# graphdeco-inria/editable-gaussian-reflections

Hardware: AMD Instinct MI355X
Metric: Mrays/s fwd+bwd @1080p, 1M Gaussians (higher is better)
Workload: dtype f32; 1 GPU; BASELINE config C: synthetic dense-init room+spheres cloud, HEADLINE variant = init (literal dense-init opacity 0.1 (config.py:44): Kc ~ 22 per ray, bounces mostly die), N=1000000, 1920x1080, one training iteration: export + update_bvh + forward + backward + grad import, num_bounces=2, jitter on, reference default config; variant=init, gaussians=1000000, width=1920, height=1080, parallelism=image tiles x1 + 1 all-reduce of the launch's [22N] gradients, team_help=product default (on)

## Files before the change

### editable-gaussian-reflections_amd/csrc/backward_chain.hpp

```cpp
#pragma once

constexpr int BOUNCE_QUEUE_FLOATS = 25 * EGR_WAVE;
static_assert(EGR_GT_STRIDE * EGR_GT_SLOTS >= BOUNCE_QUEUE_FLOATS, "the bounce queues must fit into the table");

template <int TEAM> struct BwdWave {
    int lane, wv;
    uint32_t *gt_keys;
    float *gt_vals;
    uint32_t *gt_claim;
    float4 *stage;
    BwdTeamShared<TEAM> &bteam;
    uint4 *bitems;
    float *bdl;
    float *bray;
    float exp_power;
    int num_bounces;
    float view_size;
    uint32_t bepoch;
    bool table_dirty;
};

struct BwdDiag {
    EGR_TIMES(unsigned long long bw_t0 = 0ull, bw_t1 = 0ull; uint32_t bw_rows0 = 0u;)
};

struct RayGrads {
    f3 dL_rgb, dL_n, dL_f0;
    float dL_depth, dL_rough;
    f3 ro, rd;
    f3 rem_rgb, rem_n, rem_f0;
    float rem_depth, rem_rough, T_minus_Ttot;
};

template <bool PRIMARY, bool BATCH, int TEAM>
EGR_DI RayGrads output_gradients(const DeviceView &v, const BwdWave<TEAM> &W, const ChainTask &task, const TaskGeom &tg, const StateRef &S, const int step,
                                 const uint32_t steps_done, const uint32_t nhits) {
    RayGrads g{mk3(0, 0, 0), mk3(0, 0, 0), mk3(0, 0, 0), 0.0f, 0.0f, mk3(0, 0, 0), mk3(0, 0, 1), mk3(0, 0, 0), mk3(0, 0, 0), mk3(0, 0, 0), 0.0f, 0.0f, 0.0f};
    if (nhits > 0) {
        const uint32_t pid = tg.pixel_id;
        const float third = 1.0f / 3.0f;
        if constexpr (PRIMARY) {
            f3 o_rgb = S.ld3(SF(0, S_RGB)), o_n = S.ld3(SF(0, S_NORMAL)), o_f0 = S.ld3(SF(0, S_F0));
            float o_depth = S.ld(SF(0, S_DEPTH)), o_rough = S.ld(SF(0, S_ROUGH));
            if constexpr (BATCH) {
                const size_t P = v.num_pixels;
                const uint32_t bframe = task.bframe;
                auto tgt = [&](int b, uint32_t ch, uint32_t c) { const float *p = v.batch_targets[b]; return p ? p[((size_t)bframe * ch + c) * P + pid] : 0.0f; };
                g.dL_rgb = mk3(third * sign1(o_rgb.x - tgt(0, 3, 0)), third * sign1(o_rgb.y - tgt(0, 3, 1)), third * sign1(o_rgb.z - tgt(0, 3, 2))) * *v.cfg.loss_weight_diffuse;
                g.dL_depth = sign1(o_depth - tgt(2, 1, 0)) * *v.cfg.loss_weight_depth;
                g.dL_n = mk3(third * sign1(o_n.x - tgt(3, 3, 0)), third * sign1(o_n.y - tgt(3, 3, 1)), third * sign1(o_n.z - tgt(3, 3, 2))) * *v.cfg.loss_weight_normal;
                g.dL_f0 = mk3(third * sign1(o_f0.x - tgt(5, 3, 0)), third * sign1(o_f0.y - tgt(5, 3, 1)), third * sign1(o_f0.z - tgt(5, 3, 2))) * *v.cfg.loss_weight_f0;
                g.dL_rough = sign1(o_rough - tgt(4, 1, 0)) * *v.cfg.loss_weight_roughness;
            } else {
                const bool planes = v.target_planes != 0u;
                const size_t cs = planes ? (size_t)v.num_pixels : (size_t)1;
                auto tgt = [&](int b, uint32_t ch, uint32_t c) { const float *p = v.batch_targets[b]; return p ? p[(size_t)pid * (planes ? 1u : ch) + c * cs] : 0.0f; };
                g.dL_rgb = mk3(third * sign1(o_rgb.x - tgt(0, 3, 0)), third * sign1(o_rgb.y - tgt(0, 3, 1)), third * sign1(o_rgb.z - tgt(0, 3, 2))) * *v.cfg.loss_weight_diffuse;
                g.dL_depth = sign1(o_depth - tgt(2, 1, 0)) * *v.cfg.loss_weight_depth;
                g.dL_n = mk3(third * sign1(o_n.x - tgt(3, 3, 0)), third * sign1(o_n.y - tgt(3, 3, 1)), third * sign1(o_n.z - tgt(3, 3, 2))) * *v.cfg.loss_weight_normal;
                g.dL_f0 = mk3(third * sign1(o_f0.x - tgt(5, 3, 0)), third * sign1(o_f0.y - tgt(5, 3, 1)), third * sign1(o_f0.z - tgt(5, 3, 2))) * *v.cfg.loss_weight_f0;
                g.dL_rough = sign1(o_rough - tgt(4, 1, 0)) * *v.cfg.loss_weight_roughness;
            }
            const PrimaryRay p = primary_ray<BATCH>(v, tg, task, W.view_size);
            g.ro = p.ro, g.rd = p.rd;
        } else {
            f3 spec = mk3(0, 0, 0);
            for (int j = 1; j < W.num_bounces + 1; j++)
                if ((uint32_t)j < steps_done) spec = spec + S.ld3(SF(j, S_RGB));
            f3 t_spec;
            if constexpr (BATCH) {
                const float *p = v.batch_targets[1];
                const size_t P = v.num_pixels, q = (size_t)task.bframe * 3 * P + pid;
                t_spec = p ? mk3(p[q], p[q + P], p[q + 2 * P]) : mk3(0, 0, 0);
            } else {
                const float *p = v.batch_targets[1];
                const size_t q = (size_t)pid * (v.target_planes ? 1u : 3u), cs = v.target_planes ? (size_t)v.num_pixels : (size_t)1;
                t_spec = p ? mk3(p[q], p[q + cs], p[q + 2 * cs]) : mk3(0, 0, 0);
            }
            float down = powf(1.0f - S.ld(SF(step - 1, S_ROUGH)), EGR_ROUGHNESS_DOWNWEIGHT_GRAD_POWER);
            g.dL_rgb = (mk3(third * sign1(spec.x - t_spec.x), third * sign1(spec.y - t_spec.y), third * sign1(spec.z - t_spec.z)) *
                        *v.cfg.loss_weight_specular) * down;
            g.dL_rgb = g.dL_rgb * S.ld3(SF(step - 1, S_THR));
            g.ro = S.ld3(SF(step - 1, S_NEXT_O));
            g.rd = S.ld3(SF(step - 1, S_NEXT_D));
        }
        g.rem_rgb = S.ld3(SF(step, S_REM_RGB)), g.rem_n = S.ld3(SF(step, S_REM_NORMAL)), g.rem_f0 = S.ld3(SF(step, S_REM_F0));
        g.rem_depth = S.ld(SF(step, S_REM_DEPTH)), g.rem_rough = S.ld(SF(step, S_REM_ROUGH));
        g.T_minus_Ttot = S.ld(SF(step, S_T)) - S.ld(SF(step, S_TTOT));
    }
    return g;
}

template <int TEAM> EGR_DI uint32_t bounce_hits(const DeviceView &v, BwdWave<TEAM> &W, const RayGrads &g, uint32_t blk, const uint32_t nhits, const uint32_t max_hits) {
    const int lane = W.lane, wv = W.wv;
    const float exp_power = W.exp_power;
    BwdTeamShared<TEAM> &bteam = W.bteam;
    uint4 *const bitems = W.bitems;
    float *const bdl = W.bdl, *const bray = W.bray;
    float4 *const stage = W.stage;
    const f3 dL_rgb = g.dL_rgb, ro = g.ro, rd = g.rd, rem_rgb = g.rem_rgb;
    const float T_minus_Ttot = g.T_minus_Ttot;
    uint32_t records = 0u;
    W.table_dirty = true;
    bdl[lane] = dL_rgb.x, bdl[EGR_WAVE + lane] = dL_rgb.y, bdl[2 * EGR_WAVE + lane] = dL_rgb.z;
    bray[lane] = ro.x, bray[EGR_WAVE + lane] = ro.y, bray[2 * EGR_WAVE + lane] = ro.z, bray[3 * EGR_WAVE + lane] = rd.x, bray[4 * EGR_WAVE + lane] = rd.y, bray[5 * EGR_WAVE + lane] = rd.z;
    f3 prev_rgb = mk3(0, 0, 0), w_rgb = mk3(0, 0, 0);
    const uint32_t nblocks = (max_hits + EGR_HIT_BLOCK_ROWS - 1) / EGR_HIT_BLOCK_ROWS;
    EGR_BWD_SYNC();
    for (uint32_t b = nblocks; b-- > 0;) {
        const float4 *rows = v.hit_arena + (size_t)blk * (EGR_HIT_BLOCK_ROWS + 1) * EGR_WAVE;
        for (int chunk = EGR_HIT_BLOCK_ROWS / 4 - 1; chunk >= 0; chunk--) {
            uint32_t nitems = 0u;
            float4 rec4[4], a04[4];
#pragma unroll
            for (int r4 = 0; r4 < 4; r4++) rec4[r4] = rows[(size_t)(1 + 4 * chunk + r4) * EGR_WAVE + lane];
#pragma unroll
            for (int r4 = 0; r4 < 4; r4++) a04[r4] = v.app[2 * ((b * EGR_HIT_BLOCK_ROWS + (uint32_t)(4 * chunk + r4)) < nhits ? f2u(rec4[r4].x) : 0u)];
#pragma unroll
            for (int r4 = 3; r4 >= 0; r4--) {
                const int row = 4 * chunk + r4;
                const uint32_t it = b * EGR_HIT_BLOCK_ROWS + (uint32_t)row;
                const bool act = it < nhits;
                float dL_dalpha = 0.0f, weight = 0.0f;
                uint32_t pos = 0u;
                if (act) {
                    const float4 rec = rec4[r4];
                    pos = f2u(rec.x);
                    const float alpha = rec.z, transmittance = rec.w;
                    weight = (float)((double)transmittance / (1.0 - (double)alpha) * (double)alpha);
                    const float4 a0 = a04[r4];
                    const f3 g_rgb = mk3(a0.x, a0.y, a0.z);
                    w_rgb = w_rgb + (g_rgb - prev_rgb) * transmittance;
                    prev_rgb = g_rgb;
                    const float one_m_alpha = 1.0f - alpha, r1ma = egr_rcp_refined(one_m_alpha);
                    const float tmp1 = egr_div_rn(1.0f, one_m_alpha, r1ma);
                    dL_dalpha += dot(w_rgb * tmp1, dL_rgb);
                    const float tmp2 = -egr_div_rn(T_minus_Ttot, one_m_alpha, r1ma);
                    dL_dalpha += tmp2 * dot(rem_rgb, dL_rgb);
                }
                const unsigned long long am = __ballot(act);
                if (act) bitems[nitems + __builtin_amdgcn_mbcnt_hi((uint32_t)(am >> 32), __builtin_amdgcn_mbcnt_lo((uint32_t)am, 0u))] = make_uint4((uint32_t)lane, f2u(dL_dalpha), pos, f2u(weight));
                nitems += (uint32_t)__popcll(am);
            }
            if (nitems == 0u) continue;
            EGR_BWD_SYNC();
            const uint32_t nbatch = (nitems + (uint32_t)EGR_WAVE - 1u) / (uint32_t)EGR_WAVE;
            if constexpr (TEAM > 1) {
                if (lane == 0) {
                    lds_poke(&bteam.finished[wv], 0u);
                    lds_poke(&bteam.nitems[wv], nitems);
                    W.bepoch = (W.bepoch + 1u) & 0xFFFu;
                    lds_poke(&bteam.ticket[wv], (W.bepoch << 20) | (nbatch << 10));
                }
                for (;;) {
                    uint32_t tk = 0u;
                    if (lane == 0) tk = atomicAdd(&bteam.ticket[wv], 1u);
                    tk = uniform_u32(tk);
                    const uint32_t bi = tk & 0x3FFu;
                    if (bi >= nbatch) break;
                    records += bounce_batch(v, exp_power, bitems, bdl, bray, bi * (uint32_t)EGR_WAVE, nitems, stage, lane);
                    if (lane == 0) atomicAdd(&bteam.finished[wv], 1u);
                }
                while (uniform_u32(lds_peek(&bteam.finished[wv])) < nbatch) __builtin_amdgcn_s_sleep(1);
            } else {
                for (uint32_t bi = 0; bi < nbatch; bi++) records += bounce_batch(v, exp_power, bitems, bdl, bray, bi * (uint32_t)EGR_WAVE, nitems, stage, lane);
            }
            EGR_BWD_SYNC();
        }
        blk = f2u(rows[0].x);
    }
    return records;
}

template <int TEAM> EGR_DI uint32_t primary_hits(const DeviceView &v, BwdWave<TEAM> &W, const RayGrads &g, uint32_t blk, const uint32_t nhits, const uint32_t max_hits) {
    const int lane = W.lane;
    uint32_t *const gt_keys = W.gt_keys, *const gt_claim = W.gt_claim;
    float *const gt_vals = W.gt_vals;
    float4 *const stage = W.stage;
    const f3 dL_rgb = g.dL_rgb, dL_n = g.dL_n, dL_f0 = g.dL_f0, ro = g.ro, rd = g.rd, rem_rgb = g.rem_rgb, rem_n = g.rem_n, rem_f0 = g.rem_f0;
    const float dL_depth = g.dL_depth, dL_rough = g.dL_rough, rem_depth = g.rem_depth, rem_rough = g.rem_rough, T_minus_Ttot = g.T_minus_Ttot;
    uint32_t records = 0u;
    f3 prev_rgb = mk3(0, 0, 0), w_rgb = mk3(0, 0, 0), prev_n = mk3(0, 0, 0), w_n = mk3(0, 0, 0), prev_f0 = mk3(0, 0, 0), w_f0 = mk3(0, 0, 0);
    float prev_rough = 0, w_rough = 0, prev_depth = 0, w_depth = 0;
    const uint32_t nblocks = (max_hits + EGR_HIT_BLOCK_ROWS - 1) / EGR_HIT_BLOCK_ROWS;
    EGR_STATS(unsigned long long bt_math = 0ull, bt_table = 0ull, bt_wide = 0ull, bt_rows = 0ull;)
    for (uint32_t b = nblocks; b-- > 0;) {
        const float4 *rows = v.hit_arena + (size_t)blk * (EGR_HIT_BLOCK_ROWS + 1) * EGR_WAVE;
        int pf_row = -1;
        float4 rec_pf = make_float4(0.f, 0.f, 0.f, 0.f);
        for (int row = EGR_HIT_BLOCK_ROWS - 1; row >= 0; row--) {
            const uint32_t it = b * EGR_HIT_BLOCK_ROWS + (uint32_t)row;
            if (it >= max_hits) continue;
            bool direct = false, want = false;
            uint32_t dpos = 0;
            float gx[EGR_GT_COMPS];
            EGR_STATS(const unsigned long long bt0 = __builtin_amdgcn_s_memtime(); unsigned long long bt1 = bt0; bt_rows++;)
            float4 rec_cur = rec_pf;
            const bool have_pf = pf_row == row;
            if (row > 0) {
                if (it <= nhits) rec_pf = rows[(size_t)row * EGR_WAVE + lane];
                pf_row = row - 1;
            }
            if (!have_pf) {
                if (it < nhits) rec_cur = rows[(size_t)(1 + row) * EGR_WAVE + lane];
#if defined(__HIP_DEVICE_COMPILE__)
                asm volatile("" ::"v"(rec_cur.x), "v"(rec_cur.y), "v"(rec_cur.z), "v"(rec_cur.w));
#endif
            }
            if (it < nhits) {
                const float4 rec = rec_cur;
                const uint32_t pos = f2u(rec.x);
                const float distance = rec.y, alpha = rec.z, transmittance = rec.w;
                const float4 a0 = v.app[2 * pos], a1 = v.app[2 * pos + 1], a2 = v.inst_w[4 * pos + 3];
                const f3 g_rgb = mk3(a0.x, a0.y, a0.z);
                const float weight = (float)((double)transmittance / (1.0 - (double)alpha) * (double)alpha);
                f3 d_rgb = (dL_rgb * weight);
                f3 d_n = dL_n * weight, d_f0 = dL_f0 * weight;
                float d_rough = dL_rough * weight;

                w_rgb = w_rgb + (g_rgb - prev_rgb) * transmittance;
                prev_rgb = g_rgb;
                {
                    f3 g_n = mk3(a0.w, a1.x, a1.y), g_f0 = mk3(a1.z, a1.w, a2.x);
                    w_n = w_n + (g_n - prev_n) * transmittance;
                    prev_n = g_n;
                    w_f0 = w_f0 + (g_f0 - prev_f0) * transmittance;
                    prev_f0 = g_f0;
                    w_rough += (a2.y - prev_rough) * transmittance;
                    prev_rough = a2.y;
                    w_depth += (distance - prev_depth) * transmittance;
                    prev_depth = distance;
                }
                float dL_dalpha = 0.0f;
                const float one_m_alpha = 1.0f - alpha, r1ma = egr_rcp_refined(one_m_alpha);
                const float tmp1 = egr_div_rn(1.0f, one_m_alpha, r1ma);
                dL_dalpha += dot(w_rgb * tmp1, dL_rgb);
                dL_dalpha += dot(w_n * tmp1, dL_n);
                dL_dalpha += dot(w_f0 * tmp1, dL_f0);
                dL_dalpha += (w_rough * tmp1) * dL_rough;
                dL_dalpha += (w_depth * tmp1) * dL_depth;
                const float tmp2 = -egr_div_rn(T_minus_Ttot, one_m_alpha, r1ma);
                dL_dalpha += tmp2 * dot(rem_rgb, dL_rgb);
                dL_dalpha += tmp2 * dot(rem_n, dL_n);
                dL_dalpha += tmp2 * dot(rem_f0, dL_f0);
                dL_dalpha += tmp2 * (rem_rough * dL_rough);
                dL_dalpha += tmp2 * (rem_depth * dL_depth);

                hit_geometry_fn(v, W.exp_power, pos, a2, ro, rd, dL_dalpha, gx);
                gx[PC_RGB] = d_rgb.x, gx[PC_RGB + 1] = d_rgb.y, gx[PC_RGB + 2] = d_rgb.z, gx[PC_WEIGHT] = weight;
                gx[PC_NORMAL] = d_n.x, gx[PC_NORMAL + 1] = d_n.y, gx[PC_NORMAL + 2] = d_n.z;
                gx[PC_F0] = d_f0.x, gx[PC_F0 + 1] = d_f0.y, gx[PC_F0 + 2] = d_f0.z, gx[PC_ROUGH] = d_rough;
                EGR_STATS(bt1 = __builtin_amdgcn_s_memtime();)
                dpos = pos;
                want = primary_presum(pos, gx, lane);
            }
            direct = primary_table_add(v, want, dpos, gx, gt_keys, gt_vals, gt_claim, stage, lane, records);
            EGR_STATS(const unsigned long long bt2 = __builtin_amdgcn_s_memtime(); bt_math += bt1 - bt0; bt_table += bt2 - bt1;)
            if (__ballot(direct) != 0ull) {
                float lo[EGR_REC0_COMPS], hi[EGR_REC1_COMPS];
#pragma unroll
                for (int c = 0; c < EGR_REC0_COMPS; c++) lo[c] = gx[c];
#pragma unroll
                for (int c = 0; c < EGR_REC1_COMPS; c++) hi[c] = gx[EGR_REC0_COMPS + c];
                wide_add_wave<EGR_REC0_CELL>(v, direct, dpos, lo, stage);
                wide_add_wave<EGR_REC1_CELL>(v, direct, dpos, hi, stage);
                records += 2u * (uint32_t)__popcll(__ballot(direct));
            }
            EGR_STATS(bt_wide += __builtin_amdgcn_s_memtime() - bt2;)
        }
        blk = f2u(rows[0].x);
    }
    EGR_STATS(const unsigned long long bt3 = __builtin_amdgcn_s_memtime();)
    records += grad_table_flush(v, gt_keys, gt_vals, stage, lane);
    EGR_STATS(if (lane == 0) {
        unsigned long long *d = diag64(v.control, DG_BWD_MATH_CYC);
        atomicAdd(d, bt_math), atomicAdd(d + 1, bt_table), atomicAdd(d + 2, bt_wide), atomicAdd(d + 3, __builtin_amdgcn_s_memtime() - bt3), atomicAdd(d + 4, bt_rows);
    })
    return records;
}

template <bool PRIMARY, int TEAM, bool BATCH> EGR_DI uint32_t backward_step(const DeviceView &v, BwdWave<TEAM> &W, const uint32_t tq, const int step, BwdDiag &D) {
    const int lane = W.lane;
    const uint32_t tqo = v.bwd_order[tq];
    const uint32_t blk = v.task_last_block[(size_t)step * (BATCH ? v.num_tasks * v.batch_frames : v.num_tasks) + tqo];
    if (blk == 0xFFFFFFFFu) return 0u;
    const ChainTask task = decode_task<BATCH>(v, tqo);
    const TaskGeom tg = task_geom(v, task.tb, lane);
    const StateRef S = state_of(v, task.tq, lane);
    const uint32_t steps_done = tg.inside ? f2u(S.ld(F_STEPS)) : 0u;
    const uint32_t nhits = (tg.inside && (uint32_t)step < steps_done && blk != 0xFFFFFFFFu) ? f2u(S.ld(SF(step, S_NHITS))) : 0u;
    const uint32_t max_hits = wave_max_u32(nhits);
    if (max_hits == 0) return 0u;
    EGR_TIMES_IS(8, if (PRIMARY) D.bw_rows0 = max_hits;)
    const RayGrads g = output_gradients<PRIMARY, BATCH>(v, W, task, tg, S, step, steps_done, nhits);
    if constexpr (PRIMARY) return primary_hits(v, W, g, blk, nhits, max_hits);
    else return bounce_hits(v, W, g, blk, nhits, max_hits);
}

template <int TEAM, bool BATCH> EGR_DI void backward_chain(const DeviceView v) {
    const int lane = threadIdx.x & (EGR_WAVE - 1);
    const int wv = __builtin_amdgcn_readfirstlane((int)(threadIdx.x >> 6));
    __shared__ uint32_t gt_keys_all[TEAM][EGR_GT_SLOTS];
    __shared__ __attribute__((aligned(16))) float gt_vals_all[TEAM][EGR_GT_STRIDE * EGR_GT_SLOTS];
    __shared__ uint32_t gt_claim_all[TEAM][EGR_GT_SLOTS];
    __shared__ float4 stage_all[TEAM][4 * EGR_WAVE];
    __shared__ BwdTeamShared<TEAM> bteam;
    if (threadIdx.x == 0) bteam.done = 0u;
    if (threadIdx.x < TEAM) bteam.ticket[threadIdx.x] = 0u, bteam.nitems[threadIdx.x] = 0u, bteam.finished[threadIdx.x] = 0u;
    uint32_t *const gt_keys = gt_keys_all[wv];
    float *const gt_vals = gt_vals_all[wv];
    for (int s = lane; s < EGR_GT_SLOTS; s += EGR_WAVE) gt_keys[s] = EGR_GT_EMPTY;
    for (int s = lane; s < EGR_GT_STRIDE * EGR_GT_SLOTS; s += EGR_WAVE) gt_vals[s] = 0.0f;
    __syncthreads();
    const float exp_power = *v.cfg.exp_power;
    const int num_bounces = min(*v.cfg.num_bounces, EGR_MAX_BOUNCES);
    const float view_size = BATCH ? 0.0f : tanf(*v.cam.vertical_fov_radians / 2.0f);
    BwdWave<TEAM> W{lane, wv, gt_keys, gt_vals, gt_claim_all[wv], stage_all[wv], bteam, reinterpret_cast<uint4 *>(gt_vals), gt_vals + 16 * EGR_WAVE, gt_vals + 19 * EGR_WAVE,
                    exp_power, num_bounces, view_size, 0u, false};
    uint32_t cur_q = blockIdx.x & 7u;
    uint32_t records = 0u;

    for (;;) {
        const uint32_t tq = wave_next_task(v.queues + 8 * EGR_QUEUE_STRIDE, BATCH ? v.num_tasks * v.batch_frames : v.num_tasks, cur_q, lane);
        if (tq == 0xFFFFFFFFu) break;
        BwdDiag D;
        EGR_TIMES_IS(8, D.bw_t0 = __builtin_amdgcn_s_memrealtime();)
        W.table_dirty = false;
        records += backward_step<true, TEAM, BATCH>(v, W, tq, 0, D);
        EGR_TIMES_IS(8, D.bw_t1 = __builtin_amdgcn_s_memrealtime();)
        for (int step = num_bounces; step >= 1; step--) records += backward_step<false, TEAM, BATCH>(v, W, tq, step, D);
        if (W.table_dirty) {
            EGR_BWD_SYNC();
            for (int s = lane; s < BOUNCE_QUEUE_FLOATS; s += EGR_WAVE) gt_vals[s] = 0.0f;
            EGR_BWD_SYNC();
        }
        EGR_TIMES_IS(8,
            const unsigned long long bw_t2 = __builtin_amdgcn_s_memrealtime();
            const TaskGeom btg = task_geom(v, decode_task<BATCH>(v, v.bwd_order[tq]).tb, lane);
            if (btg.inside) {
                if (lane == 0) v.stats.num_traversed_per_pixel[btg.pixel_id] = EGR_STAMP31(D.bw_t0), v.stats.num_accumulated_per_pixel[btg.pixel_id] = EGR_STAMP31(bw_t2);
                if (lane == 1) v.stats.num_traversed_per_pixel[btg.pixel_id] = EGR_STAMP31(D.bw_t1), v.stats.num_accumulated_per_pixel[btg.pixel_id] = (int32_t)D.bw_rows0;
            })
    }
    if constexpr (TEAM > 1) {
        if (lane == 0) atomicAdd(&bteam.done, 1u);
        records += bwd_team_help<TEAM>(v, exp_power, bteam, gt_vals_all, W.stage, wv, lane);
    }
    if (lane == 0 && records) atomicAdd(v.control + CW_BUCKET_RECORDS, records);
}
```

### editable-gaussian-reflections_amd/csrc/trace.hip

```cpp
#include <algorithm>
#include <cstdio>
#include <cstdlib>
#include <type_traits>
#include <utility>
#include <vector>

#define EGR_CONTRACT_AFTER_EPILOGUE
#include "egr_diag.hpp"
#include "egr_epilogue.hpp"

#ifndef EGR_GPOP
#define EGR_GPOP 5
#endif
#define EGR_WALK_MAX_LEAVES (8 * EGR_GPOP * EGR_WIDTH)
#define EGR_LBUF (64 + 2 * EGR_WALK_MAX_LEAVES)
#ifndef EGR_FPOP
#define EGR_FPOP 2
#endif
#ifndef EGR_PSTK
#define EGR_PSTK 512
#endif

namespace {

// ... 722 lines not shown
            float *cell = gt_vals + slot * EGR_GT_STRIDE;
            float cur[EGR_GT_COMPS];
#pragma unroll
            for (int c = 0; c < EGR_GT_COMPS; c++) cur[c] = cell[c];
#pragma unroll
            for (int c = 0; c < EGR_GT_COMPS; c++) cell[c] = cur[c] + gx[c];
            pending = false;
        }
        EGR_BWD_SYNC();
    }
    return want && !found;
}

struct ChainVec { double x, y, z; };
EGR_DI void scale_rot_chain(const float4 &M0, const float4 &M1, const float4 &M2, const float4 &qu, const float sigma, const float eps, const ChainVec &dl2w0, const ChainVec &dl2w1,
                            const ChainVec &dl2w2, double (&d_scale)[3], double (&d_rot)[4]) {
    using T = double;
    const T scaling_factor = sigma, eps_scale_grad = eps;
    const ChainVec scaling = {T(M0.w), T(M1.w), T(M2.w)};
    const ChainVec den = {scaling.x * scaling_factor + eps_scale_grad, scaling.y * scaling_factor + eps_scale_grad, scaling.z * scaling_factor + eps_scale_grad};
    auto div3 = [&](const float4 &m) { return ChainVec{T(m.x) / den.x, T(m.y) / den.y, T(m.z) / den.z}; };
    const ChainVec rot_0 = div3(M0), rot_1 = div3(M1), rot_2 = div3(M2);
    d_scale[0] = (dl2w0.x * rot_0.x + dl2w1.x * rot_1.x + dl2w2.x * rot_2.x) * scaling.x;
    d_scale[1] = (dl2w0.y * rot_0.y + dl2w1.y * rot_1.y + dl2w2.y * rot_2.y) * scaling.y;
    d_scale[2] = (dl2w0.z * rot_0.z + dl2w1.z * rot_1.z + dl2w2.z * rot_2.z) * scaling.z;
    auto mul3 = [](const ChainVec &a, const ChainVec &b) { return ChainVec{a.x * b.x, a.y * b.y, a.z * b.z}; };
    const ChainVec dr0 = mul3(dl2w0, scaling), dr1 = mul3(dl2w1, scaling), dr2 = mul3(dl2w2, scaling);
    const T qr = qu.x, qx = qu.y, qy = qu.z, qz = qu.w;
    const T qn = sqrt(qr * qr + qx * qx + qy * qy + qz * qz);
    const T r = qr / qn, x = qx / qn, y = qy / qn, z = qz / qn;
    const T dL_dr = T(2) * x * (dr2.y - dr1.z) + T(2) * y * (dr0.z - dr2.x) + T(2) * z * (dr1.x - dr0.y);
    const T dL_dx = T(-4) * x * (dr1.y + dr2.z) + T(2) * y * (dr0.y + dr1.x) + T(2) * z * (dr0.z + dr2.x) + T(2) * r * (dr2.y - dr1.z);
    const T dL_dy = T(2) * x * (dr0.y + dr1.x) - T(4) * y * (dr0.x + dr2.z) + T(2) * z * (dr1.z + dr2.y) + T(2) * r * (dr0.z - dr2.x);
    const T dL_dz = T(2) * x * (dr0.z + dr2.x) + T(2) * y * (dr1.z + dr2.y) - T(4) * z * (dr0.x + dr1.y) + T(2) * r * (dr1.x - dr0.y);
    const T dd = dL_dr * qr + dL_dx * qx + dL_dy * qy + dL_dz * qz;
    const T qn3 = qn * qn * qn;
    const T inv3 = T(1) / qn3, inv1 = T(1) / qn;
    d_rot[0] = dd * -qr * inv3 + dL_dr * inv1, d_rot[1] = dd * -qx * inv3 + dL_dx * inv1;
    d_rot[2] = dd * -qy * inv3 + dL_dy * inv1, d_rot[3] = dd * -qz * inv3 + dL_dz * inv1;
}

template <class GX> EGR_DI void hit_geometry_fn(const DeviceView &v, const float exp_power, uint32_t pos, const float4 &a2, const f3 &ro, const f3 &rd, float dL_dalpha, GX &gx) {
    const float opacity = a2.z, scaling_factor = a2.w;
    const float4 W0 = v.inst_w[4 * pos], W1 = v.inst_w[4 * pos + 1], W2 = v.inst_w[4 * pos + 2];
    f3 lo, ld, dhat, u;
    float t_unused;
    bool behind_unused, outside_unused;
    candidate_geometry(W0, W1, W2, ro, rd, lo, ld, dhat, t_unused, u, behind_unused, outside_unused);
    const f3 local_hit = u * scaling_factor;
    const float sq_norm = dot(local_hit, local_hit);
    const float gaussval = egr_gaussian_sq(sq_norm, exp_power);

    float d_opacity = EGR_MAX_ALPHA * dL_dalpha * gaussval;
    d_opacity = d_opacity * opacity * (1.0f - opacity);
    const float dL_dgaussval = EGR_MAX_ALPHA * dL_dalpha * opacity;
    const float dL_dsq_norm = gaussval * pow_exp_m1(sq_norm, exp_power);
    const f3 dL_dx_local = (-local_hit * dL_dsq_norm) * dL_dgaussval;
    const f3 dL_dx_world = mk3(dot(mk3(W0.x, W1.x, W2.x), dL_dx_local), dot(mk3(W0.y, W1.y, W2.y), dL_dx_local),
                               dot(mk3(W0.z, W1.z, W2.z), dL_dx_local)) * scaling_factor;
    const f3 d_mean = -dL_dx_world;
    gx[PC_OPA] = d_opacity, gx[PC_MEAN] = d_mean.x, gx[PC_MEAN + 1] = d_mean.y, gx[PC_MEAN + 2] = d_mean.z;
    const f3 ql = -dL_dx_local * scaling_factor;
    gx[PC_Q] = ql.x * local_hit.x, gx[PC_Q + 1] = ql.x * local_hit.y, gx[PC_Q + 2] = ql.x * local_hit.z;
    gx[PC_Q + 3] = ql.y * local_hit.y, gx[PC_Q + 4] = ql.y * local_hit.z, gx[PC_Q + 5] = ql.z * local_hit.z;
}

EGR_DI uint32_t bounce_batch(const DeviceView &v, const float exp_power, const uint4 *bitems, const float *bdl, const float *bray, uint32_t i0, uint32_t nitems, float4 *stage, int lane) {
    static_assert(PC_OPA == GC_OPA && PC_MEAN == GC_MEAN && PC_RGB == GC_RGB && PC_WEIGHT == GC_WEIGHT && PC_Q == GC_Q && GC_Q + 6 == EGR_REC0_COMPS, "components 0-13 of a hit are segment 0 of the row");
    const bool valid = i0 + (uint32_t)lane < nitems;
    uint32_t dpos = 0;
    float gx[EGR_REC0_COMPS];
#pragma unroll
    for (int c = 0; c < EGR_REC0_COMPS; c++) gx[c] = 0.0f;
    if (valid) {
        const uint4 item = bitems[i0 + (uint32_t)lane];
        const uint32_t ray = item.x, pos = item.z;
        const float weight = u2f(item.w);
        const float4 a2 = v.inst_w[4 * pos + 3];
        const f3 iro = mk3(bray[ray], bray[EGR_WAVE + ray], bray[2 * EGR_WAVE + ray]), ird = mk3(bray[3 * EGR_WAVE + ray], bray[4 * EGR_WAVE + ray], bray[5 * EGR_WAVE + ray]);
        hit_geometry_fn(v, exp_power, pos, a2, iro, ird, u2f(item.y), gx);
        gx[GC_RGB] = bdl[ray] * weight, gx[GC_RGB + 1] = bdl[EGR_WAVE + ray] * weight, gx[GC_RGB + 2] = bdl[2 * EGR_WAVE + ray] * weight;
        gx[GC_WEIGHT] = weight;
        dpos = pos;
    }
    wide_add_wave<EGR_REC0_CELL>(v, valid, dpos, gx, stage);
    return (uint32_t)__popcll(__ballot(valid));
}

#ifndef EGR_BWD_TEAM
#define EGR_BWD_TEAM 4
#endif
template <int TEAM> struct BwdTeamShared {
    uint32_t done;
    uint32_t ticket[TEAM], nitems[TEAM], finished[TEAM];
};

#ifndef EGR_BWD_WAVES
#define EGR_BWD_WAVES 3
#endif
#ifndef EGR_ORDER_BUCKETS
#define EGR_ORDER_BUCKETS 16
#endif
#ifndef EGR_ORDER_SHIFT
#define EGR_ORDER_SHIFT 7
#endif
__global__ void __launch_bounds__(256) k_order_backward(DeviceView v) {
    __shared__ uint32_t cnt[EGR_ORDER_BUCKETS][256 + 1];
    const uint32_t chunk = ((v.num_tasks + 7u) / 8u + 3u) & ~3u, q = blockIdx.x;
    const uint32_t beg = q * chunk, end = min(beg + chunk, v.num_tasks);
    if (beg >= end) return;
    const uint32_t t = threadIdx.x, n = end - beg, per = (n + 255u) / 256u;
    const uint32_t i0 = min(t * per, n), i1 = min(i0 + per, n);
    auto bucket = [](uint32_t cost) { return (uint32_t)EGR_ORDER_BUCKETS - 1u - min(cost >> EGR_ORDER_SHIFT, (uint32_t)EGR_ORDER_BUCKETS - 1u); };
    for (int b = 0; b < EGR_ORDER_BUCKETS; b++) cnt[b][t] = 0u;
    for (uint32_t i = i0; i < i1; i++) cnt[bucket(v.task_cost[beg + i])][t]++;
    __syncthreads();
    if (t < (uint32_t)EGR_ORDER_BUCKETS) {
        uint32_t acc = 0u;
        for (int j = 0; j < 256; j++) {
            const uint32_t c = cnt[t][j];
            cnt[t][j] = acc, acc += c;
        }
        cnt[t][256] = acc;
    }
    __syncthreads();
    uint32_t start[EGR_ORDER_BUCKETS];
    uint32_t acc = 0u;
#pragma unroll
    for (int b = 0; b < EGR_ORDER_BUCKETS; b++) start[b] = acc + cnt[b][t], acc += cnt[b][256];
    for (uint32_t i = i0; i < i1; i++) {
        const uint32_t bk = bucket(v.task_cost[beg + i]);
        uint32_t at = 0u;
#pragma unroll
        for (int b = 0; b < EGR_ORDER_BUCKETS; b++)
            if ((uint32_t)b == bk) at = start[b]++;
        v.bwd_order[beg + at] = beg + i;
    }
}

template <int TEAM> EGR_DI uint32_t bwd_team_help(const DeviceView &v, const float exp_power, BwdTeamShared<TEAM> &bteam, float (*gt_vals_all)[EGR_GT_STRIDE * EGR_GT_SLOTS],
                                                  float4 *stage, const int wv, const int lane) {
    uint32_t records = 0u;
    while (uniform_u32(lds_peek(&bteam.done)) < (uint32_t)TEAM) {
        bool any = false;
        for (int dlt = 1; dlt < TEAM; dlt++) {
            const int w = (wv + dlt) % TEAM;
            const uint32_t peek = uniform_u32(lds_peek(&bteam.ticket[w]));
            if ((peek & 0x3FFu) >= ((peek >> 10) & 0x3FFu)) continue;
            uint32_t tk = 0u;
            if (lane == 0) tk = atomicAdd(&bteam.ticket[w], 1u);
            tk = uniform_u32(tk);
            const uint32_t bi = tk & 0x3FFu, nbatch = (tk >> 10) & 0x3FFu;
            if (bi >= nbatch) continue;
            const uint32_t nitems = uniform_u32(lds_peek(&bteam.nitems[w]));
            const uint4 *bitems = reinterpret_cast<const uint4 *>(gt_vals_all[w]);
            records += bounce_batch(v, exp_power, bitems, gt_vals_all[w] + 16 * EGR_WAVE, gt_vals_all[w] + 19 * EGR_WAVE, bi * (uint32_t)EGR_WAVE, nitems, stage, lane);
            if (lane == 0) atomicAdd(&bteam.finished[w], 1u);
            any = true;
        }
        if (!any) __builtin_amdgcn_s_sleep(2);
    }
    return records;
}

#include "backward_chain.hpp"
template <int TEAM> __global__ void __launch_bounds__(EGR_WAVE * TEAM) __attribute__((amdgpu_waves_per_eu(EGR_BWD_WAVES, EGR_BWD_WAVES))) k_backward_chain(DeviceView v) {
    backward_chain<TEAM, false>(v);
}
template <int TEAM> __global__ void __launch_bounds__(EGR_WAVE * TEAM) __attribute__((amdgpu_waves_per_eu(EGR_BWD_WAVES, EGR_BWD_WAVES))) k_backward_batch(DeviceView v) {
    backward_chain<TEAM, true>(v);
}

template <bool OVERWRITE> EGR_DI void grad_gather_row(const DeviceView &v, const uint32_t gid) {
    const size_t pos = v.pos_of_gid[gid];
    float4 *row = reinterpret_cast<float4 *>(v.grad_rows + pos * EGR_ROW_STRIDE);
    float x[EGR_ROW_STRIDE];
    uint32_t any = 0, any_l = 0;
#pragma unroll
    for (int q = 0; q < EGR_ROW_STRIDE / 4; q++) {
        const float4 r = row[q];
        x[4 * q] = r.x, x[4 * q + 1] = r.y, x[4 * q + 2] = r.z, x[4 * q + 3] = r.w;
        any |= (f2u(r.x) | f2u(r.y) | f2u(r.z) | f2u(r.w)) << 1;
    }
    if (!OVERWRITE && any == 0) return;
    if (any != 0) {
#pragma unroll
        for (int q = 0; q < EGR_ROW_STRIDE / 4; q++) row[q] = make_float4(0.f, 0.f, 0.f, 0.f);
    }
#pragma unroll
    for (int c = 0; c < 6; c++) any_l |= f2u(x[GC_Q + c]) << 1;
    float d_scale[3] = {0.f, 0.f, 0.f}, d_rot[4] = {0.f, 0.f, 0.f, 0.f};
    if (any_l != 0) {
        const float4 *im = v.inst_m + 4 * (size_t)gid;
        const float4 M0 = im[0], M1 = im[1], M2 = im[2], qu = im[3];
        const float4 W0 = v.inst_w[4 * pos], W1 = v.inst_w[4 * pos + 1], W2 = v.inst_w[4 * pos + 2];
        const float scaling_factor = v.inst_w[4 * pos + 3].w;
        const double q00 = x[GC_Q], q01 = x[GC_Q + 1], q02 = x[GC_Q + 2], q11 = x[GC_Q + 3], q12 = x[GC_Q + 4], q22 = x[GC_Q + 5];
        auto dl2w_of = [&](double w0, double w1, double w2) { return ChainVec{w0 * q00 + w1 * q01 + w2 * q02, w0 * q01 + w1 * q11 + w2 * q12, w0 * q02 + w1 * q12 + w2 * q22}; };
        double ds[3], dr[4];
        scale_rot_chain(M0, M1, M2, qu, scaling_factor, *v.cfg.eps_scale_grad, dl2w_of(W0.x, W1.x, W2.x), dl2w_of(W0.y, W1.y, W2.y), dl2w_of(W0.z, W1.z, W2.z), ds, dr);
#pragma unroll
        for (int a = 0; a < 3; a++) d_scale[a] = (float)ds[a];
#pragma unroll
        for (int a = 0; a < 4; a++) d_rot[a] = (float)dr[a];
    }
    const egr_gaussians &g = v.g;
    auto put = [](float *p, float val) {
        if (OVERWRITE) *p = val;
        else *p += val;
    };
    put(g.dL_dopacity + gid, x[GC_OPA]);
#pragma unroll
    for (int a = 0; a < 3; a++) {
        put(g.dL_dscale + 3 * gid + a, d_scale[a]), put(g.dL_dmean + 3 * gid + a, x[GC_MEAN + a]), put(g.dL_drgb + 3 * gid + a, x[GC_RGB + a]);
        put(g.dL_dnormal + 3 * gid + a, x[GC_NORMAL + a]), put(g.dL_df0 + 3 * gid + a, x[GC_F0 + a]);
    }
#pragma unroll
    for (int a = 0; a < 4; a++) put(g.dL_drotation + 4 * gid + a, d_rot[a]);
    put(g.dL_droughness + gid, x[GC_ROUGH]);
    put(g.total_weight + gid, x[GC_WEIGHT]);
}
EGR_DI void import_block_tensor(float *__restrict__ to, const float *from, const uint32_t block, const uint32_t n, const uint32_t width) {
    const size_t beg = (size_t)block * 256u * width, end = min(beg + (size_t)256u * width, (size_t)n * width);
    if (end - beg == (size_t)256u * width && ((reinterpret_cast<uintptr_t>(to) | reinterpret_cast<uintptr_t>(from)) & 15u) == 0) {
        float4 *to4 = reinterpret_cast<float4 *>(to + beg);
        const float4 *from4 = reinterpret_cast<const float4 *>(from + beg);
        for (uint32_t q = threadIdx.x; q < 64u * width; q += 256u) {
            float4 a = to4[q];
            const float4 b = from4[q];
            a.x += b.x, a.y += b.y, a.z += b.z, a.w += b.w;
            to4[q] = a;
        }
    } else {
        for (size_t j = beg + threadIdx.x; j < end; j += 256u) to[j] += from[j];
    }
}
template <bool OVERWRITE, bool IMPORT> __global__ void __launch_bounds__(256) k_grad_gather(DeviceView v, EgrGradImport imp) {
    static_assert(!(OVERWRITE && IMPORT), "an importing launch adds");
    const uint32_t gid = blockIdx.x * 256 + threadIdx.x;
    if constexpr (!IMPORT) {
        if (gid >= v.n) return;
        grad_gather_row<OVERWRITE>(v, gid);
    } else {
        if (gid < v.n) grad_gather_row<false>(v, gid);
        __syncthreads();
        const egr_gaussians &g = v.g;
        import_block_tensor(imp.dL_drgb, g.dL_drgb, blockIdx.x, v.n, 3), import_block_tensor(imp.dL_dnormal, g.dL_dnormal, blockIdx.x, v.n, 3);
        import_block_tensor(imp.dL_df0, g.dL_df0, blockIdx.x, v.n, 3), import_block_tensor(imp.dL_droughness, g.dL_droughness, blockIdx.x, v.n, 1);
        import_block_tensor(imp.dL_dopacity, g.dL_dopacity, blockIdx.x, v.n, 1), import_block_tensor(imp.dL_dscale, g.dL_dscale, blockIdx.x, v.n, 3);
        import_block_tensor(imp.dL_dmean, g.dL_dmean, blockIdx.x, v.n, 3), import_block_tensor(imp.dL_drotation, g.dL_drotation, blockIdx.x, v.n, 4);
    }
}

__global__ void __launch_bounds__(EGR_WAVE) k_finish(DeviceView v) {
    const int lane = threadIdx.x;
    const bool accumulate = *v.cfg.accumulate_samples != 0;
    const float cnt = accumulate ? (float)(*v.fb.accumulated_sample_count + 1) : 1.0f;
    const size_t P = v.num_pixels;
    for (uint32_t task = blockIdx.x; task < v.num_tasks; task += gridDim.x) {
        const TaskGeom tg = task_geom(v, task, lane);
        if (!tg.inside) continue;
        const StateRef S = state_of(v, task, lane);
        const uint32_t steps = f2u(S.ld(F_STEPS));
        f3 final = mk3(0, 0, 0);
        for (int s = 0; s < EGR_NSTEPS; s++) {
            const bool done = (uint32_t)s < steps;
            f3 rgb = done ? S.ld3(SF(s, S_RGB)) : mk3(0, 0, 0), n = done ? S.ld3(SF(s, S_NORMAL)) : mk3(0, 0, 0);
            f3 f0 = done ? S.ld3(SF(s, S_F0)) : mk3(0, 0, 0);
            float depth = done ? S.ld(SF(s, S_DEPTH)) : 0.0f, rough = done ? S.ld(SF(s, S_ROUGH)) : 0.0f;
            float T = done ? S.ld(SF(s, S_T)) : 1.0f, Ttot = done ? S.ld(SF(s, S_TTOT)) : 1.0f;
            f3 no = done ? S.ld3(SF(s, S_NEXT_O)) : mk3(0, 0, 0), nd = done ? S.ld3(SF(s, S_NEXT_D)) : mk3(0, 0, 0);
            const size_t q = tg.pixel_id + P * (size_t)s;
            if (accumulate) {
#define EGR_ACC3(buf, val) { float *a_ = v.fb.buf + 3 * q; a_[0] += val.x, a_[1] += val.y, a_[2] += val.z; val = div_s(mk3(a_[0], a_[1], a_[2]), cnt); }
#define EGR_ACC1(buf, val) { float *a_ = v.fb.buf + q; a_[0] += val; val = a_[0] / cnt; }
                EGR_ACC3(accumulated_rgb, rgb) EGR_ACC1(accumulated_transmittance, T) EGR_ACC1(accumulated_total_transmittance, Ttot)
                EGR_ACC1(accumulated_depth, depth) EGR_ACC3(accumulated_normal, n) EGR_ACC3(accumulated_f0, f0) EGR_ACC1(accumulated_roughness, rough)
#undef EGR_ACC3
#undef EGR_ACC1
            }
            final = final + rgb;
            float *o;
            o = v.fb.output_rgb + 3 * q, o[0] = rgb.x, o[1] = rgb.y, o[2] = rgb.z;
            o = v.fb.output_normal + 3 * q, o[0] = n.x, o[1] = n.y, o[2] = n.z;
            o = v.fb.output_f0 + 3 * q, o[0] = f0.x, o[1] = f0.y, o[2] = f0.z;
            o = v.fb.output_ray_origin + 3 * q, o[0] = no.x, o[1] = no.y, o[2] = no.z;
            o = v.fb.output_ray_direction + 3 * q, o[0] = nd.x, o[1] = nd.y, o[2] = nd.z;
            v.fb.output_depth[q] = depth, v.fb.output_roughness[q] = rough;
            v.fb.output_transmittance[q] = T, v.fb.output_total_transmittance[q] = Ttot;
        }
        float *o = v.fb.output_final + 3 * (size_t)tg.pixel_id;
        o[0] = final.x, o[1] = final.y, o[2] = final.z;
    }
}

__global__ void k_batch_cameras(const float *__restrict__ R, const float *__restrict__ centre, const float *__restrict__ fov, uint32_t views, float znear, float zfar,
                                float *__restrict__ table) {
    const uint32_t i = blockIdx.x * blockDim.x + threadIdx.x;
    if (i == views) table[(size_t)views * EGR_BATCH_CAM_FLOATS] = znear, table[(size_t)views * EGR_BATCH_CAM_FLOATS + 1] = zfar;
    if (i >= views) return;
    float *rec = table + (size_t)i * EGR_BATCH_CAM_FLOATS;
    const float *r9 = R + 9 * (size_t)i;
    for (int t = 0; t < 9; t++) {
        const int r = t / 3, c = t % 3;
        rec[3 + 3 * c + r] = c == 0 ? r9[t] : -r9[t];
    }
    for (int a = 0; a < 3; a++) rec[a] = centre[3 * (size_t)i + a];
    rec[12] = tanf(fov[i] / 2.0f);
    rec[13] = rec[14] = rec[15] = 0.0f;
// ... 596 lines not shown
```

Measured before the change: 485.9 Mrays/s.

## Batch bounce-hit queue with leftover carry and adaptive chunk rows

Restructures the backward bounce-hit loop so a partial batch of queued items (the remainder below a full wave) carries over to the next chunk instead of being flushed as a partly empty batch. When few rays in the wave are live, it queues eight rows per chunk instead of four. Both aim to fill bounce batches more densely and to cut the number of syncs and team ticket rounds. The team ticket now encodes an offset and total span, and the epoch is kept in LDS. The cost is more complex queue bookkeeping, an extra ballot pass to check whether the next chunk fits, and reliance on static capacity bounds.

```diff
diff --git a/editable-gaussian-reflections_amd/csrc/backward_chain.hpp b/editable-gaussian-reflections_amd/csrc/backward_chain.hpp
--- a/editable-gaussian-reflections_amd/csrc/backward_chain.hpp
+++ b/editable-gaussian-reflections_amd/csrc/backward_chain.hpp
@@ -16,7 +16,6 @@
     float exp_power;
     int num_bounces;
     float view_size;
-    uint32_t bepoch;
     bool table_dirty;
 };
 
@@ -91,85 +90,123 @@
     return g;
 }
 
-template <int TEAM> EGR_DI uint32_t bounce_hits(const DeviceView &v, BwdWave<TEAM> &W, const RayGrads &g, uint32_t blk, const uint32_t nhits, const uint32_t max_hits) {
+constexpr int BOUNCE_QUEUE_ITEMS = 4 * EGR_WAVE;
+constexpr int BOUNCE_ROWS_SHORT = 4, BOUNCE_ROWS_LONG = EGR_HIT_BLOCK_ROWS;
+constexpr int BOUNCE_LONG_MAX_RAYS = (BOUNCE_QUEUE_ITEMS - (EGR_WAVE - 1)) / BOUNCE_ROWS_LONG;
+static_assert(BOUNCE_QUEUE_ITEMS * 4 == 16 * EGR_WAVE && BOUNCE_QUEUE_ITEMS * 4 + 9 * EGR_WAVE == BOUNCE_QUEUE_FLOATS, "queue, radiance gradients and rays are the bounce steps' part of the table");
+static_assert(EGR_HIT_BLOCK_ROWS % BOUNCE_ROWS_SHORT == 0 && BOUNCE_ROWS_SHORT * EGR_WAVE <= BOUNCE_QUEUE_ITEMS &&
+                  BOUNCE_ROWS_LONG * BOUNCE_LONG_MAX_RAYS + (EGR_WAVE - 1) <= BOUNCE_QUEUE_ITEMS,
+              "a chunk never queues more than the queue holds: four rows of 64 rays without a leftover (a leftover is carried only where it fits), eight rows of the live rays behind any leftover");
+static_assert(BOUNCE_QUEUE_ITEMS / EGR_WAVE < 0x3FF, "a chunk's batches fit the ticket's 10-bit fields");
+
+EGR_DI uint32_t bounce_queue_chunk(const DeviceView &v, const int R, const float4 *rows, const int row0, const uint32_t it0, const uint32_t nhits, const f3 &dL_rgb, const f3 &rem_rgb,
+                                   const float T_minus_Ttot, f3 &prev_rgb, f3 &w_rgb, uint4 *bitems, uint32_t nitems, const int lane) {
+    struct { float x, z, w; } rec4[BOUNCE_ROWS_LONG];
+    f3 a04[BOUNCE_ROWS_LONG];
+#pragma unroll
+    for (int r4 = 0; r4 < BOUNCE_ROWS_LONG; r4++) {
+        if (r4 >= R) break;
+        const float *rp = reinterpret_cast<const float *>(rows + (size_t)(1 + row0 + r4) * EGR_WAVE + lane);
+        rec4[r4].x = rp[0], rec4[r4].z = rp[2], rec4[r4].w = rp[3];
+    }
+#pragma unroll
+    for (int r4 = 0; r4 < BOUNCE_ROWS_LONG; r4++) {
+        if (r4 >= R) break;
+        const float *a = reinterpret_cast<const float *>(v.app + 2 * ((it0 + (uint32_t)r4) < nhits ? f2u(rec4[r4].x) : 0u));
+        a04[r4] = mk3(a[0], a[1], a[2]);
+    }
+#pragma unroll
+    for (int r4 = BOUNCE_ROWS_LONG - 1; r4 >= 0; r4--) {
+        if (r4 >= R) continue;
+        const bool act = it0 + (uint32_t)r4 < nhits;
+        float dL_dalpha = 0.0f, weight = 0.0f;
+        uint32_t pos = 0u;
+        if (act) {
+            pos = f2u(rec4[r4].x);
+            const float alpha = rec4[r4].z, transmittance = rec4[r4].w;
+            weight = (float)((double)transmittance / (1.0 - (double)alpha) * (double)alpha);
+            const f3 g_rgb = a04[r4];
+            w_rgb = w_rgb + (g_rgb - prev_rgb) * transmittance;
+            prev_rgb = g_rgb;
+            const float one_m_alpha = 1.0f - alpha, r1ma = egr_rcp_refined(one_m_alpha);
+            const float tmp1 = egr_div_rn(1.0f, one_m_alpha, r1ma);
+            dL_dalpha += dot(w_rgb * tmp1, dL_rgb);
+            const float tmp2 = -egr_div_rn(T_minus_Ttot, one_m_alpha, r1ma);
+            dL_dalpha += tmp2 * dot(rem_rgb, dL_rgb);
+        }
+        const unsigned long long am = __ballot(act);
+        if (act) bitems[nitems + __builtin_amdgcn_mbcnt_hi((uint32_t)(am >> 32), __builtin_amdgcn_mbcnt_lo((uint32_t)am, 0u))] = make_uint4((uint32_t)lane, f2u(dL_dalpha), pos, f2u(weight));
+        nitems += (uint32_t)__popcll(am);
+    }
+    return nitems;
+}
+
+template <int TEAM> EGR_DI uint32_t bounce_chunks(const DeviceView &v, BwdWave<TEAM> &W, const int R, const RayGrads &g, uint32_t blk, const uint32_t nhits, const uint32_t max_hits) {
     const int lane = W.lane, wv = W.wv;
     const float exp_power = W.exp_power;
     BwdTeamShared<TEAM> &bteam = W.bteam;
     uint4 *const bitems = W.bitems;
     float *const bdl = W.bdl, *const bray = W.bray;
     float4 *const stage = W.stage;
-    const f3 dL_rgb = g.dL_rgb, ro = g.ro, rd = g.rd, rem_rgb = g.rem_rgb;
+    const f3 dL_rgb = g.dL_rgb, rem_rgb = g.rem_rgb;
     const float T_minus_Ttot = g.T_minus_Ttot;
     uint32_t records = 0u;
-    W.table_dirty = true;
-    bdl[lane] = dL_rgb.x, bdl[EGR_WAVE + lane] = dL_rgb.y, bdl[2 * EGR_WAVE + lane] = dL_rgb.z;
-    bray[lane] = ro.x, bray[EGR_WAVE + lane] = ro.y, bray[2 * EGR_WAVE + lane] = ro.z, bray[3 * EGR_WAVE + lane] = rd.x, bray[4 * EGR_WAVE + lane] = rd.y, bray[5 * EGR_WAVE + lane] = rd.z;
     f3 prev_rgb = mk3(0, 0, 0), w_rgb = mk3(0, 0, 0);
     const uint32_t nblocks = (max_hits + EGR_HIT_BLOCK_ROWS - 1) / EGR_HIT_BLOCK_ROWS;
-    EGR_BWD_SYNC();
+    uint32_t left = 0u;
     for (uint32_t b = nblocks; b-- > 0;) {
         const float4 *rows = v.hit_arena + (size_t)blk * (EGR_HIT_BLOCK_ROWS + 1) * EGR_WAVE;
-        for (int chunk = EGR_HIT_BLOCK_ROWS / 4 - 1; chunk >= 0; chunk--) {
-            uint32_t nitems = 0u;
-            float4 rec4[4], a04[4];
-#pragma unroll
-            for (int r4 = 0; r4 < 4; r4++) rec4[r4] = rows[(size_t)(1 + 4 * chunk + r4) * EGR_WAVE + lane];
-#pragma unroll
-            for (int r4 = 0; r4 < 4; r4++) a04[r4] = v.app[2 * ((b * EGR_HIT_BLOCK_ROWS + (uint32_t)(4 * chunk + r4)) < nhits ? f2u(rec4[r4].x) : 0u)];
-#pragma unroll
-            for (int r4 = 3; r4 >= 0; r4--) {
-                const int row = 4 * chunk + r4;
-                const uint32_t it = b * EGR_HIT_BLOCK_ROWS + (uint32_t)row;
-                const bool act = it < nhits;
-                float dL_dalpha = 0.0f, weight = 0.0f;
-                uint32_t pos = 0u;
-                if (act) {
-                    const float4 rec = rec4[r4];
-                    pos = f2u(rec.x);
-                    const float alpha = rec.z, transmittance = rec.w;
-                    weight = (float)((double)transmittance / (1.0 - (double)alpha) * (double)alpha);
-                    const float4 a0 = a04[r4];
-                    const f3 g_rgb = mk3(a0.x, a0.y, a0.z);
-                    w_rgb = w_rgb + (g_rgb - prev_rgb) * transmittance;
-                    prev_rgb = g_rgb;
-                    const float one_m_alpha = 1.0f - alpha, r1ma = egr_rcp_refined(one_m_alpha);
-                    const float tmp1 = egr_div_rn(1.0f, one_m_alpha, r1ma);
-                    dL_dalpha += dot(w_rgb * tmp1, dL_rgb);
-                    const float tmp2 = -egr_div_rn(T_minus_Ttot, one_m_alpha, r1ma);
-                    dL_dalpha += tmp2 * dot(rem_rgb, dL_rgb);
-                }
-                const unsigned long long am = __ballot(act);
-                if (act) bitems[nitems + __builtin_amdgcn_mbcnt_hi((uint32_t)(am >> 32), __builtin_amdgcn_mbcnt_lo((uint32_t)am, 0u))] = make_uint4((uint32_t)lane, f2u(dL_dalpha), pos, f2u(weight));
-                nitems += (uint32_t)__popcll(am);
-            }
-            if (nitems == 0u) continue;
+        for (int row0 = EGR_HIT_BLOCK_ROWS - R; row0 >= 0; row0 -= R) {
+            const uint32_t it0 = b * EGR_HIT_BLOCK_ROWS + (uint32_t)row0;
+            if (it0 >= max_hits) continue;
+            const uint32_t total = bounce_queue_chunk(v, R, rows, row0, it0, nhits, dL_rgb, rem_rgb, T_minus_Ttot, prev_rgb, w_rgb, bitems, left, lane);
+            bool carry = it0 != 0u;
+            if (R != BOUNCE_ROWS_LONG && carry) {
+                uint32_t next = 0u;
+                for (int r = 1; r <= R; r++) next += (uint32_t)__popcll(__ballot(it0 - (uint32_t)r < nhits));
+                carry = (total & (uint32_t)(EGR_WAVE - 1)) + next <= (uint32_t)BOUNCE_QUEUE_ITEMS;
+            }
+            left = carry ? total & (uint32_t)(EGR_WAVE - 1) : 0u;
+            if (left == total) continue;
             EGR_BWD_SYNC();
-            const uint32_t nbatch = (nitems + (uint32_t)EGR_WAVE - 1u) / (uint32_t)EGR_WAVE;
             if constexpr (TEAM > 1) {
+                const uint32_t nbatch = (total - left + (uint32_t)EGR_WAVE - 1u) / (uint32_t)EGR_WAVE;
                 if (lane == 0) {
                     lds_poke(&bteam.finished[wv], 0u);
-                    lds_poke(&bteam.nitems[wv], nitems);
-                    W.bepoch = (W.bepoch + 1u) & 0xFFFu;
-                    lds_poke(&bteam.ticket[wv], (W.bepoch << 20) | (nbatch << 10));
+                    lds_poke(&bteam.nitems[wv], (left << 16) | total);
+                    const uint32_t epoch = ((lds_peek(&bteam.ticket[wv]) >> 20) + 1u) & 0xFFFu;
+                    lds_poke(&bteam.ticket[wv], (epoch << 20) | (nbatch << 10));
                 }
                 for (;;) {
                     uint32_t tk = 0u;
                     if (lane == 0) tk = atomicAdd(&bteam.ticket[wv], 1u);
                     tk = uniform_u32(tk);
-                    const uint32_t bi = tk & 0x3FFu;
-                    if (bi >= nbatch) break;
-                    records += bounce_batch(v, exp_power, bitems, bdl, bray, bi * (uint32_t)EGR_WAVE, nitems, stage, lane);
+                    const uint32_t i0 = left + (tk & 0x3FFu) * (uint32_t)EGR_WAVE;
+                    if (i0 >= total) break;
+                    records += bounce_batch(v, exp_power, bitems, bdl, bray, i0, total, stage, lane);
                     if (lane == 0) atomicAdd(&bteam.finished[wv], 1u);
                 }
-                while (uniform_u32(lds_peek(&bteam.finished[wv])) < nbatch) __builtin_amdgcn_s_sleep(1);
+                while (left + uniform_u32(lds_peek(&bteam.finished[wv])) * (uint32_t)EGR_WAVE < total) __builtin_amdgcn_s_sleep(1);
             } else {
-                for (uint32_t bi = 0; bi < nbatch; bi++) records += bounce_batch(v, exp_power, bitems, bdl, bray, bi * (uint32_t)EGR_WAVE, nitems, stage, lane);
+                for (uint32_t i0 = left; i0 < total; i0 += (uint32_t)EGR_WAVE) records += bounce_batch(v, exp_power, bitems, bdl, bray, i0, total, stage, lane);
             }
             EGR_BWD_SYNC();
         }
         blk = f2u(rows[0].x);
     }
     return records;
+}
+
+template <int TEAM> EGR_DI uint32_t bounce_hits(const DeviceView &v, BwdWave<TEAM> &W, const RayGrads &g, const uint32_t blk, const uint32_t nhits, const uint32_t max_hits) {
+    const int lane = W.lane;
+    float *const bdl = W.bdl, *const bray = W.bray;
+    const f3 dL_rgb = g.dL_rgb, ro = g.ro, rd = g.rd;
+    W.table_dirty = true;
+    bdl[lane] = dL_rgb.x, bdl[EGR_WAVE + lane] = dL_rgb.y, bdl[2 * EGR_WAVE + lane] = dL_rgb.z;
+    bray[lane] = ro.x, bray[EGR_WAVE + lane] = ro.y, bray[2 * EGR_WAVE + lane] = ro.z, bray[3 * EGR_WAVE + lane] = rd.x, bray[4 * EGR_WAVE + lane] = rd.y, bray[5 * EGR_WAVE + lane] = rd.z;
+    EGR_BWD_SYNC();
+    const int R = (uint32_t)__popcll(__ballot(nhits > 0u)) <= (uint32_t)BOUNCE_LONG_MAX_RAYS ? BOUNCE_ROWS_LONG : BOUNCE_ROWS_SHORT;
+    return bounce_chunks<TEAM>(v, W, R, g, blk, nhits, max_hits);
 }
 
 template <int TEAM> EGR_DI uint32_t primary_hits(const DeviceView &v, BwdWave<TEAM> &W, const RayGrads &g, uint32_t blk, const uint32_t nhits, const uint32_t max_hits) {
@@ -316,7 +353,7 @@
     const int num_bounces = min(*v.cfg.num_bounces, EGR_MAX_BOUNCES);
     const float view_size = BATCH ? 0.0f : tanf(*v.cam.vertical_fov_radians / 2.0f);
     BwdWave<TEAM> W{lane, wv, gt_keys, gt_vals, gt_claim_all[wv], stage_all[wv], bteam, reinterpret_cast<uint4 *>(gt_vals), gt_vals + 16 * EGR_WAVE, gt_vals + 19 * EGR_WAVE,
-                    exp_power, num_bounces, view_size, 0u, false};
+                    exp_power, num_bounces, view_size, false};
     uint32_t cur_q = blockIdx.x & 7u;
     uint32_t records = 0u;
 
diff --git a/editable-gaussian-reflections_amd/csrc/trace.hip b/editable-gaussian-reflections_amd/csrc/trace.hip
--- a/editable-gaussian-reflections_amd/csrc/trace.hip
+++ b/editable-gaussian-reflections_amd/csrc/trace.hip
@@ -898,9 +898,9 @@
             tk = uniform_u32(tk);
             const uint32_t bi = tk & 0x3FFu, nbatch = (tk >> 10) & 0x3FFu;
             if (bi >= nbatch) continue;
-            const uint32_t nitems = uniform_u32(lds_peek(&bteam.nitems[w]));
+            const uint32_t span = uniform_u32(lds_peek(&bteam.nitems[w]));
             const uint4 *bitems = reinterpret_cast<const uint4 *>(gt_vals_all[w]);
-            records += bounce_batch(v, exp_power, bitems, gt_vals_all[w] + 16 * EGR_WAVE, gt_vals_all[w] + 19 * EGR_WAVE, bi * (uint32_t)EGR_WAVE, nitems, stage, lane);
+            records += bounce_batch(v, exp_power, bitems, gt_vals_all[w] + 16 * EGR_WAVE, gt_vals_all[w] + 19 * EGR_WAVE, (span >> 16) + bi * (uint32_t)EGR_WAVE, span & 0xFFFFu, stage, lane);
             if (lane == 0) atomicAdd(&bteam.finished[w], 1u);
             any = true;
         }
```

Result: no change. 488.7 Mrays/s (median of 6 runs) (+0.6%).
